# BienLuky/Rectified-SpaAttn

Measured on AMD Instinct MI355X. Metric: attention-layer TFLOPs/sec (rectified block-sparse attention, HunyuanVideo seq~120k d=128 bf16), higher is better.
Workload: dtype bf16; 1 GPU; hunyuan_720p_128f: B=1 H=24 S=115456 (115200 visual + 256 text, 200 valid) D=128, top_k=90, regime=r2 (p_remain=0.0, neighbors=none); heads_per_gpu=24, parallelism=head-shard x1, world_size=1

## Files before the change

### rectified_spaattn_amd/csrc/rsa_attn.h

```cpp
#pragma once
#include <string.h>

#include <type_traits>

#include "rsa_common.h"

typedef short s16x4 __attribute__((ext_vector_type(4)));
typedef short s16x8 __attribute__((ext_vector_type(8)));
typedef __bf16 bf16x8 __attribute__((ext_vector_type(8)));
typedef _Float16 f16x8 __attribute__((ext_vector_type(8)));
typedef float f32x16 __attribute__((ext_vector_type(16)));
typedef float f32x4 __attribute__((ext_vector_type(4)));

template <typename Tag>
struct Elem;
template <>
struct Elem<bf16_tag> {
    static __device__ __forceinline__ f32x16 mfma(s16x8 a, s16x8 b, f32x16 c) {
        return __builtin_amdgcn_mfma_f32_32x32x16_bf16(__builtin_bit_cast(bf16x8, a), __builtin_bit_cast(bf16x8, b),
                                                       c, 0, 0, 0);
    }
    static __device__ __forceinline__ unsigned short from_f32(float f) {
        return __builtin_bit_cast(unsigned short, (__bf16)f);
    }
    static __device__ __forceinline__ s16x8 cvt8(const float* f) {
        bf16x8 r;
#pragma unroll
        for (int i = 0; i < 8; ++i) r[i] = (__bf16)f[i];
        return __builtin_bit_cast(s16x8, r);
    }
};
template <>
struct Elem<fp16_tag> {
    static __device__ __forceinline__ f32x16 mfma(s16x8 a, s16x8 b, f32x16 c) {
        return __builtin_amdgcn_mfma_f32_32x32x16_f16(__builtin_bit_cast(f16x8, a), __builtin_bit_cast(f16x8, b), c,
                                                      0, 0, 0);
    }
    static __device__ __forceinline__ unsigned short from_f32(float f) {
        return __builtin_bit_cast(unsigned short, (_Float16)f);
    }
    static __device__ __forceinline__ s16x8 cvt8(const float* f) {
        f16x8 r;
#pragma unroll
        for (int i = 0; i < 8; ++i) r[i] = (_Float16)f[i];
        return __builtin_bit_cast(s16x8, r);
    }
};

enum { MODE_SPARSE = 0, MODE_DENSE = 1 };

struct WalkArgs {
    unsigned short* out;
    long osb, osh, oss;
    const int32_t* cols;
    const int32_t* counts;
    const float* R;
    const float* comp;
    float* tpart;
    float* tail_part;
    unsigned* gsync;
    int mode, H, Sq, Sk;
    int NBv, NQB, NB_total;
    int kv_valid, kv_text_valid, q_text_end;
    int q_split, kv_split;
    int causal;
    int n_heavy_pad, NBp, BH;
    int tsplit, tper;
    int heavy_last;
    int tail_first, tail_n, tail_p;
    int gsync_gen;
    int gsync_ratio;
    int k5_static;
};

struct AttnArgs : WalkArgs {
    const unsigned short *q, *k, *v;
    long qsb, qsh, qss, ksb, ksh, kss, vsb, vsh, vss;
    float qk_scale;
    int rows256;
    int blk;
    int txt0;
    const int32_t* row_lo;
    const int32_t* row_hi;
    long range_sb;
    int kv_group, list_group, gqa;
};
enum { RSA_GQA_NONE = 0, RSA_GQA_HEAD = 1, RSA_GQA_PAIR = 2 };

template <typename A>
__device__ __forceinline__ const A& rsa_kernargs() {
    return *static_cast<const A*>((const void*)__builtin_amdgcn_kernarg_segment_ptr());
}

__host__ __device__ __forceinline__ int rsa_walk_unit(int j, int NBp) { return (j & 7) * (NBp >> 3) + (j >> 3); }
enum { WALK_NONE = 0, WALK_SPARSE = 1, WALK_TEXT = 2 };
__device__ __forceinline__ int rsa_walk_map(const WalkArgs& a, int work, int n_units, int& bh, int& unit, int& tsp, int& tail) {
    tsp = 0;
    tail = -1;
    const int n_sparse = a.BH * a.NBp;
    const bool heavy_last = a.heavy_last != 0;
    int wh = heavy_last ? work - n_sparse : work;
    int v = heavy_last ? work : work - a.n_heavy_pad;
    bool text = heavy_last ? work >= n_sparse : work < a.n_heavy_pad;
    if (a.tail_n > 0) {
        const int tail_end = a.tail_first + a.tail_n * a.tail_p;
        text = work >= tail_end;
        wh = work - tail_end;
        if (work >= a.tail_first && !text) {
            tail = work - a.tail_first;
            v = a.tail_first + tail / a.tail_p;
            tsp = tail % a.tail_p;
        }
    }
    if (text) {
        const int ntq = a.NQB - a.NBv;
        const int per_bh = ntq * a.tsplit;
        if (ntq <= 0 || wh >= a.BH * per_bh) return WALK_NONE;
        bh = wh / per_bh;
        const int rem = wh % per_bh;
        unit = a.NBv + rem / a.tsplit;
        tsp = rem % a.tsplit;
    } else {
        bh = v / a.NBp;
        unit = rsa_walk_unit(v % a.NBp, a.NBp);
        if (unit >= n_units) return WALK_NONE;
    }
    return text ? WALK_TEXT : WALK_SPARSE;
}

__device__ __forceinline__ void rsa_walk_list(const WalkArgs& a, long rowi, int tail, int tsp, const int32_t*& list, int& n_items) {
    list = a.cols + rowi * a.NB_total;
    n_items = a.counts[rowi];
    if (tail >= 0) {
        const int per = (n_items + a.tail_p - 1) / a.tail_p, first = tsp * per;
        const int left = n_items - first;
        list += first;
        n_items = left < 0 ? 0 : (left < per ? left : per);
    }
}
__device__ __forceinline__ void rsa_walk_text(const WalkArgs& a, int blk, int tsp, int& first_blk, int& n_items) {
    n_items = (a.kv_text_valid + blk - 1) / blk;
    if (a.tsplit > 1) {
        first_blk = tsp * a.tper;
        n_items = n_items - first_blk < a.tper ? n_items - first_blk : a.tper;
        if (n_items < 0) n_items = 0;
    }
}

__device__ __forceinline__ int rsa_seg_hi(const WalkArgs& a, int row) {
    const bool s1 = row >= a.q_split;
    const int lo = s1 ? a.kv_split : 0, hi = s1 ? a.Sk : a.kv_split;
    if (!a.causal) return hi;
    const int rows = s1 ? a.Sq - a.q_split : a.q_split, rin = row - (s1 ? a.q_split : 0);
    const int lim = lo + rin + 1 + ((hi - lo) - rows);
    return lim < lo ? lo : (lim < hi ? lim : hi);
}
__device__ __forceinline__ void rsa_dense_row(const WalkArgs& a, int grow, int& lo, int& hi) {
    lo = grow < a.q_split ? 0 : a.kv_split;
    hi = rsa_seg_hi(a, grow < a.Sq ? grow : a.Sq - 1);
}
__device__ __forceinline__ void rsa_dense_tile(const WalkArgs& a, int row0, int rows, int& lo_max, int& hi_min, int& hi_max,
                                               int& first_blk, int& n_items) {
    const int row1 = row0 + rows;
    int lo_min;
    const int rlast = (row1 <= a.Sq ? row1 : a.Sq) - 1;
    if (row1 <= a.q_split) { lo_min = 0; lo_max = 0; }
    else if (row0 >= a.q_split) { lo_min = lo_max = a.kv_split; }
    else { lo_min = 0; lo_max = a.kv_split; }
    hi_min = rsa_seg_hi(a, row0);
    hi_max = rsa_seg_hi(a, rlast);
    if (row0 < a.q_split && rlast >= a.q_split) {
        const int h0 = rsa_seg_hi(a, a.q_split - 1), h1 = rsa_seg_hi(a, a.q_split);
        hi_min = hi_min < h1 ? hi_min : h1;
        hi_max = hi_max > h0 ? hi_max : h0;
    }
    first_blk = lo_min / RSA_BLOCK;
    n_items = (hi_max + RSA_BLOCK - 1) / RSA_BLOCK - first_blk;
    if (hi_max <= lo_min) n_items = 0;
}

// ... 79 lines not shown
```

### rectified_spaattn_amd/csrc/rsa_attn.hip

```cpp
#include <stdlib.h>

#include <atomic>
#include <mutex>
#include "rsa_attn.h"

static int g_k5_tsplit = 1;
extern int g_rsa_k3_prefix;
extern int g_rsa_k3_long;
extern int g_rsa_k4_split;
extern int g_rsa_k2_dma;
static int g_k5_tail_split = 1;
static int g_k5_text_last = 1;
static int g_shard_invariant = 0;
static int g_k5_gsync_ratio = 2;
int rsa_gsync_ratio() { return g_k5_gsync_ratio; }
static int g_k5_rows256 = 1;
static int g_k5_static = 1;
int rsa_k5_static() { return g_k5_static; }
static int g_k5_gqa_pair = 0;
static int g_k5_gsync = 1;

extern "C" int rsa_set_tuning(const char* key, int value) {
    static const bool enabled = [] { const char* e = getenv("RSA_TUNING"); return e && e[0] == '1'; }();
    if (!key) return RSA_ERR_BAD_ARG;
    if (!enabled) return RSA_ERR_UNSUPPORTED;
    if (strcmp(key, "k3_prefix") == 0) { g_rsa_k3_prefix = value; return RSA_OK; }
    if (strcmp(key, "k3_long") == 0) { g_rsa_k3_long = value; return RSA_OK; }
    if (strcmp(key, "k4_split") == 0) { g_rsa_k4_split = value; return RSA_OK; }
    if (strcmp(key, "k2_dma") == 0) { g_rsa_k2_dma = value; return RSA_OK; }
    if (strcmp(key, "k5_static") == 0) { g_k5_static = value; return RSA_OK; }
    if (strcmp(key, "k5_rows256") == 0) { g_k5_rows256 = value; return RSA_OK; }
    if (strcmp(key, "k5_tsplit") == 0) { g_k5_tsplit = value; return RSA_OK; }
    if (strcmp(key, "k5_gsync") == 0) { g_k5_gsync = value; return RSA_OK; }
    if (strcmp(key, "k5_gsync_ratio") == 0) { g_k5_gsync_ratio = value; return RSA_OK; }
    if (strcmp(key, "k5_text_last") == 0) { g_k5_text_last = value; return RSA_OK; }
    if (strcmp(key, "k5_tail_split") == 0) { g_k5_tail_split = value; return RSA_OK; }
    if (strcmp(key, "k5_gqa_pair") == 0) { g_k5_gqa_pair = value; return RSA_OK; }
    if (strcmp(key, "fp8_variant") == 0) { rsa_set_fp8_variant(value); return RSA_OK; }
    if (strcmp(key, "fp8_smooth_k") == 0) { rsa_set_fp8_smooth_k(value); return RSA_OK; }
    return RSA_ERR_BAD_ARG;
}

template <typename Tag>
__global__ __launch_bounds__(256) void text_combine_kernel(const float* __restrict__ tpart, unsigned short* out,
                                                           long osb, long osh, long oss, int D, int H, int txt0, int ntq,
                                                           int tsplit, int q_text_end, int Sq, long rows_total) {
    const int lane = threadIdx.x & 63;
    const long row = (long)blockIdx.x * 4 + (threadIdx.x >> 6);
    if (row >= rows_total) return;
    const long bhq = row / RSA_BLOCK;
    const int r = (int)(row % RSA_BLOCK);
    const long bh = bhq / ntq;
    const int tq = (int)(bhq % ntq);
    const int grow = txt0 + tq * RSA_BLOCK + r;
    if (grow >= Sq) return;
    const float* base = tpart + rsa_part_row(bhq * tsplit, r, D);
    const long pstride = rsa_part_row(1, 0, D);
    constexpr int MAXP = RSA_TEXT_SPLIT;
    float mv[MAXP], lv[MAXP];
#pragma unroll
    for (int s = 0; s < MAXP; ++s) {
        const int sc = s < tsplit ? s : 0;
        const float2 ml = *reinterpret_cast<const float2*>(base + sc * pstride + D);
        mv[s] = s < tsplit ? ml.x : -INFINITY;
        lv[s] = ml.y;
    }
    float M = -INFINITY;
#pragma unroll
    for (int s = 0; s < MAXP; ++s) M = fmaxf(M, mv[s]);
    float L = 0.0f;
    float acc[2] = {0.0f, 0.0f};
#pragma unroll
    for (int s0 = 0; s0 < MAXP; s0 += 8) {
        if (s0 >= tsplit) break;
        float x[8][2];
#pragma unroll
        for (int u = 0; u < 8; ++u) {
            const int sc = s0 + u < tsplit ? s0 + u : 0;
#pragma unroll
            for (int e = 0; e < 2; ++e) {
                const int d = lane + 64 * e;
                x[u][e] = d < D ? base[sc * pstride + d] : 0.0f;
            }
        }
#pragma unroll
        for (int u = 0; u < 8; ++u) {
            if (s0 + u < tsplit) {
                const float wgt = (mv[s0 + u] == -INFINITY) ? 0.0f : __builtin_amdgcn_exp2f(mv[s0 + u] - M);
                L += lv[s0 + u] * wgt;
// ... 77 lines not shown
        text_combine_kernel<fp16_tag><<<grid, 256, 0, s>>>(a.tpart, a.out, a.osb, a.osh, a.oss, D, a.H, a.NBv * blk, ntq, a.tsplit,
                                                         a.q_text_end, a.Sq, rows);
    return rsa_launch_status();
}

__device__ unsigned g_rsa_gsync[RSA_GSYNC_RING][RSA_GSYNC_SLOT_WORDS];
unsigned* rsa_gsync_slot(int which, unsigned grid, int wg_per_cu, hipStream_t s, int* gen) {
    static std::atomic<unsigned*> base[64];
    static std::atomic<unsigned> ticket{0};
    *gen = 32 * (wg_per_cu > 0 ? wg_per_cu : 2);
    if (!(g_k5_gsync & which) || wg_per_cu <= 0 || grid <= 16u * (unsigned)*gen) return nullptr;
    const unsigned gens = ((grid + 7) / 8 + *gen - 1) / *gen;
    int dev = -1;
    if (gens > RSA_GSYNC_MAXG || hipGetDevice(&dev) != hipSuccess || dev < 0 || dev >= 64) return nullptr;
    unsigned* b = base[dev].load();
    if (!b) {
        int cus = 0;
        if (hipDeviceGetAttribute(&cus, hipDeviceAttributeMultiprocessorCount, dev) != hipSuccess || cus != 256) {
            base[dev].store(reinterpret_cast<unsigned*>(1));
            return nullptr;
        }
        if (hipGetSymbolAddress(reinterpret_cast<void**>(&b), HIP_SYMBOL(g_rsa_gsync)) != hipSuccess) return nullptr;
        base[dev].store(b);
    }
    if (b == reinterpret_cast<unsigned*>(1)) return nullptr;
    unsigned* slot = b + (size_t)(ticket.fetch_add(1) % RSA_GSYNC_RING) * RSA_GSYNC_SLOT_WORDS;
    return hipMemsetAsync(slot, 0, (8 + 8 * (size_t)gens) * sizeof(unsigned), s) == hipSuccess ? slot : nullptr;
}
int rsa_wg_per_cu(const void* kernel, int block, size_t lds_bytes) {
    struct Entry { const void* k; size_t lds; int dev, n; };
    static Entry cache[64];
    static std::atomic<int> used{0};
    static std::mutex mu;
    int dev = -1;
    if (hipGetDevice(&dev) != hipSuccess) return 0;
    const int nu = used.load(std::memory_order_acquire);
    for (int i = 0; i < nu; ++i)
        if (cache[i].k == kernel && cache[i].lds == lds_bytes && cache[i].dev == dev) return cache[i].n;
    int n = 0;
    if (hipOccupancyMaxActiveBlocksPerMultiprocessor(&n, kernel, block, lds_bytes) != hipSuccess) n = 0;
    std::lock_guard<std::mutex> lk(mu);
    const int at = used.load();
    if (at < 64) { cache[at] = Entry{kernel, lds_bytes, dev, n}; used.store(at + 1, std::memory_order_release); }
    return n;
}

int rsa_plan_walk(WalkArgs& a, int BH, int D, const WalkPolicy& pol, size_t tpart_bytes, long* nblocks) {
    *nblocks = 0;
    const int blk = pol.blk;
    const int ntq = a.NQB - a.NBv;
    if (a.tpart && tpart_bytes == 0) return RSA_ERR_WORKSPACE;
    const size_t piece_bytes = (size_t)rsa_part_row(1, 0, D) * sizeof(float);
    a.BH = BH;
    a.NBp = ((blk == 64 ? (a.NBv + 1) >> 1 : a.NBv) + 7) & ~7;
    const int n_txt_items = (a.kv_text_valid + blk - 1) / blk;
    a.tsplit = 1; a.tper = n_txt_items;
    if (a.mode == MODE_SPARSE && ntq > 0 && a.tpart && g_k5_tsplit && n_txt_items >= 32) {
        const int sp = n_txt_items / 16;
        int cap = ((long)BH * a.NBp < 8 * 512 && !g_shard_invariant) ? pol.short_grid_text_cap : 16;
        const size_t room = tpart_bytes / ((size_t)BH * (size_t)ntq * piece_bytes);
        if ((size_t)cap > room) cap = (int)room;
        a.tsplit = sp > cap ? cap : sp;
        if (a.tsplit < 2) a.tsplit = 1;
        a.tper = (n_txt_items + a.tsplit - 1) / a.tsplit;
    }
    const int n_heavy = ntq > 0 ? BH * ntq * a.tsplit : 0;
    a.heavy_last = a.tsplit > 1 && g_k5_text_last;
    a.n_heavy_pad = (n_heavy + 7) & ~7;
    const long n_sparse = (long)BH * a.NBp;
    *nblocks = (long)a.n_heavy_pad + n_sparse;
    a.tail_first = a.tail_n = a.tail_p = 0; a.tail_part = nullptr;
    if (pol.tail_split && a.mode == MODE_SPARSE && a.tpart && (n_heavy == 0 || (pol.tail_beside_text && a.heavy_last)) && g_k5_tail_split &&
        !g_shard_invariant) {
        const long full = n_sparse / 512, T = n_sparse % 512;
        const long room = 512 - a.n_heavy_pad;
        const long P = T > 0 ? (room / T < 4 ? room / T : 4) : 0;
        const size_t text_pieces = (size_t)BH * (size_t)ntq * RSA_TEXT_SPLIT;
        if (full >= 1 && T > 0 && P >= 2 && (text_pieces + (size_t)(T * P)) * piece_bytes <= tpart_bytes) {
            a.tail_first = (int)(full * 512); a.tail_n = (int)T; a.tail_p = (int)P;
            a.tail_part = a.tpart + rsa_part_row((long)text_pieces, 0, D);
            *nblocks = (long)a.tail_first + (long)a.tail_n * a.tail_p + a.n_heavy_pad;
        }
    }
    if (*nblocks <= 0) { *nblocks = 0; return RSA_OK; }
    if (*nblocks > 0x7FFFFFFF) return RSA_ERR_UNSUPPORTED;
    if (a.NB_total > 8192) return RSA_ERR_UNSUPPORTED;
    return RSA_OK;
}

static int launch_attn(AttnArgs& a, int BH, int D, int dtype, size_t tpart_bytes, hipStream_t s) {
    const bool w64 = a.blk == RSA_BLOCK;
    long nblocks;
    WalkPolicy pol;
    pol.blk = a.blk;
    pol.short_grid_text_cap = RSA_TEXT_SPLIT;
    pol.tail_split = w64 && D == 128 && a.gqa != RSA_GQA_PAIR;
    pol.tail_beside_text = true;
    int st = rsa_plan_walk(a, BH, D, pol, tpart_bytes, &nblocks);
    if (st != RSA_OK || nblocks == 0) return st;
    const size_t lds_bytes = (size_t)4 * 64 * D * 2 + (((size_t)a.NB_total * 2 + 15) & ~(size_t)15);
    st = w64 ? rsa_launch_bsfwd64(a, dim3((unsigned)nblocks), lds_bytes, D, dtype, s)
             : rsa_launch_bsfwd(a, dim3((unsigned)nblocks), lds_bytes, D, dtype, s);
    return st != RSA_OK ? st : rsa_combine_walk(a, D, a.blk, dtype, s);
}

static void fill_qkv(AttnArgs& a, const rsa_tensor4& q, const rsa_tensor4& k, const rsa_tensor4& v,
                     const rsa_out4& out) {
    a.q = static_cast<const unsigned short*>(q.ptr); a.qsb = q.stride_b; a.qsh = q.stride_h; a.qss = q.stride_s;
    a.k = static_cast<const unsigned short*>(k.ptr); a.ksb = k.stride_b; a.ksh = k.stride_h; a.kss = k.stride_s;
    a.v = static_cast<const unsigned short*>(v.ptr); a.vsb = v.stride_b; a.vsh = v.stride_h; a.vss = v.stride_s;
    a.out = static_cast<unsigned short*>(out.ptr); a.osb = out.stride_b; a.osh = out.stride_h; a.oss = out.stride_s;
    a.row_lo = nullptr; a.row_hi = nullptr; a.range_sb = 0;
    a.kv_group = 1; a.list_group = 1; a.gqa = RSA_GQA_NONE;
}

int rsa_check_out(const rsa_out4& o) {
    if (!o.ptr || (reinterpret_cast<uintptr_t>(o.ptr) & 7)) return RSA_ERR_BAD_ARG;
    if ((o.stride_b % 4) || (o.stride_h % 4) || (o.stride_s % 4)) return RSA_ERR_BAD_ARG;
    return RSA_OK;
}

static int block_sparse_fwd_b(const rsa_layout* l, int blk, rsa_tensor4 q, rsa_tensor4 k, rsa_tensor4 v,
                              const rsa_buffers* buf, rsa_out4 out, void* stream) {
    int st = rsa_check_layout_b(l, blk);
    if (st != RSA_OK) return st;
    if ((st = rsa_check_tensor(q)) || (st = rsa_check_tensor(k)) || (st = rsa_check_tensor(v)) ||
        (st = rsa_check_out(out)))
        return st;
    if (!buf || (l->NBv > 0 && (!buf->cols || !buf->counts))) return RSA_ERR_BAD_ARG;
    if ((buf->R == nullptr) != (buf->comp == nullptr)) return RSA_ERR_BAD_ARG;
    AttnArgs a;
    fill_qkv(a, q, k, v, out);
    a.cols = buf->cols; a.counts = buf->counts; a.R = buf->R; a.comp = buf->comp;
    a.tpart = buf->tpart;
    a.mode = MODE_SPARSE; a.H = l->H; a.Sq = l->S; a.Sk = l->S;
    a.NBv = l->NBv; a.NQB = l->NB_total; a.NB_total = l->NB_total;
    a.blk = blk; a.txt0 = l->NBv * blk;
    if (blk == 64) a.NQB = l->NBv + (l->NB_total - l->NBv + 1) / 2;
    a.kv_valid = l->kv_valid; a.kv_text_valid = l->kv_text_valid;
    a.q_text_end = l->NBv * blk + l->q_text_valid;
    a.q_split = 0; a.kv_split = 0; a.causal = 0; a.rows256 = 0;
    a.qk_scale = (float)((1.0 / sqrt((double)l->D)) * 1.44269504);
    return launch_attn(a, l->B * l->H, l->D, l->dtype, buf->tpart_bytes, static_cast<hipStream_t>(stream));
}
extern "C" int rsa_block_sparse_fwd(const rsa_layout* l, rsa_tensor4 q, rsa_tensor4 k, rsa_tensor4 v,
                                    const rsa_buffers* buf, rsa_out4 out, void* stream) {
    return block_sparse_fwd_b(l, RSA_BLOCK, q, k, v, buf, out, stream);
}
extern "C" int rsa_block_sparse_fwd_ex(const rsa_layout_ex* lx, rsa_tensor4 q, rsa_tensor4 k, rsa_tensor4 v,
                                       const rsa_buffers* buf, rsa_out4 out, void* stream) {
    return rsa_layout_ex_ok(lx) ? block_sparse_fwd_b(&lx->base, lx->block, q, k, v, buf, out, stream) : RSA_ERR_BAD_ARG;
}
// ... 139 lines not shown
```

### rectified_spaattn_amd/csrc/rsa_attn_kernel64.hip

```cpp
#include "rsa_attn.h"
#include <atomic>
#include "rsa_attn_block64.h"

#define RSA_K5W_CL_TO RSA_K5W_CLOBBER_TMP, RSA_K5W_CLOBBER_O
#define RSA_K5V_CL_TO RSA_K5V_CLOBBER_TMP, RSA_K5V_CLOBBER_O
#define RSA_K5W_CL_LOOP RSA_K5W_CLOBBER_TMP, RSA_K5W_CLOBBER_O, RSA_K5W_CLOBBER_LOOP
#define RSA_K5V_CL_LOOP RSA_K5V_CLOBBER_TMP, RSA_K5V_CLOBBER_O, RSA_K5V_CLOBBER_LOOP
#define RSA_K5_ASM(D_, BODY, OPS, CL, ...) \
    do { \
        if constexpr ((D_) == 128) asm volatile(RSA_K5W_##BODY RSA_K5W_##OPS : RSA_K5W_##CL __VA_ARGS__); \
        else asm volatile(RSA_K5V_##BODY RSA_K5V_##OPS : RSA_K5V_##CL __VA_ARGS__); \
    } while (0)

typedef int i32x8 __attribute__((ext_vector_type(8)));
typedef unsigned u32x4 __attribute__((ext_vector_type(4)));

__device__ __forceinline__ int k5w_max(int x, int y) { return x > y ? x : y; }
__device__ __forceinline__ int k5w_wave_max(int v) {
#pragma unroll
    for (int m = 32; m >= 1; m >>= 1) v = k5w_max(v, __shfl_xor(v, m, 64));
    return v;
}

template <typename Tag, int U, int D>
__device__ __forceinline__ void k5w_block(f32x16 (&SA)[2], f32x16 (&SB)[2], const f32x16 (&nm)[2], float (&l)[2], float (&mx)[2],
                                          const i32x8& ka, const i32x8& va) {
    if constexpr (std::is_same<Tag, bf16_tag>::value) {
        if constexpr (U == 0) RSA_K5_ASM(D, BLOCK_BF16_U0, OPS, CL_TO, , "memory");
        else if constexpr (U == 1) RSA_K5_ASM(D, BLOCK_BF16_U1, OPS, CL_TO, , "memory");
        else if constexpr (U == 2) RSA_K5_ASM(D, BLOCK_BF16_U2, OPS, CL_TO, , "memory");
        else RSA_K5_ASM(D, BLOCK_BF16_U3, OPS, CL_TO, , "memory");
    } else {
        if constexpr (U == 0) RSA_K5_ASM(D, BLOCK_F16_U0, OPS, CL_TO, , "memory");
        else if constexpr (U == 1) RSA_K5_ASM(D, BLOCK_F16_U1, OPS, CL_TO, , "memory");
        else if constexpr (U == 2) RSA_K5_ASM(D, BLOCK_F16_U2, OPS, CL_TO, , "memory");
        else RSA_K5_ASM(D, BLOCK_F16_U3, OPS, CL_TO, , "memory");
    }
}

template <int Hh, int KSI, int D>
__device__ __forceinline__ void k5w_qwrite(const s16x8& f) {
#define RSA_QW(HH, KK) do { if constexpr (D == 128) asm volatile(RSA_K5W_QWRITE_H##HH##_K##KK :: "{v[96:99]}"(f) : RSA_K5W_CLOBBER_Q); \
                            else asm volatile(RSA_K5V_QWRITE_H##HH##_K##KK :: "{v[96:99]}"(f) : RSA_K5V_CLOBBER_Q); } while (0)
    if constexpr (Hh == 0) {
        if constexpr (KSI == 0) RSA_QW(0, 0); else if constexpr (KSI == 1) RSA_QW(0, 1); else if constexpr (KSI == 2) RSA_QW(0, 2);
        else if constexpr (KSI == 3) RSA_QW(0, 3); else if constexpr (KSI == 4) RSA_QW(0, 4); else if constexpr (KSI == 5) RSA_QW(0, 5);
        else if constexpr (KSI == 6) RSA_QW(0, 6); else RSA_QW(0, 7);
    } else {
        if constexpr (KSI == 0) RSA_QW(1, 0); else if constexpr (KSI == 1) RSA_QW(1, 1); else if constexpr (KSI == 2) RSA_QW(1, 2);
        else if constexpr (KSI == 3) RSA_QW(1, 3); else if constexpr (KSI == 4) RSA_QW(1, 4); else if constexpr (KSI == 5) RSA_QW(1, 5);
        else if constexpr (KSI == 6) RSA_QW(1, 6); else RSA_QW(1, 7);
    }
#undef RSA_QW
}
template <int Hh, int DTI, int D>
__device__ __forceinline__ f32x16 k5w_oread() {
    f32x16 t;
#define RSA_OR(HH, DD) do { if constexpr (D == 128) asm volatile(RSA_K5W_OREAD_H##HH##_D##DD : "={v[96:111]}"(t)); \
                            else asm volatile(RSA_K5V_OREAD_H##HH##_D##DD : "={v[96:111]}"(t)); } while (0)
    if constexpr (Hh == 0) {
        if constexpr (DTI == 0) RSA_OR(0, 0); else if constexpr (DTI == 1) RSA_OR(0, 1); else if constexpr (DTI == 2) RSA_OR(0, 2); else RSA_OR(0, 3);
    } else {
        if constexpr (DTI == 0) RSA_OR(1, 0); else if constexpr (DTI == 1) RSA_OR(1, 1); else if constexpr (DTI == 2) RSA_OR(1, 2); else RSA_OR(1, 3);
    }
#undef RSA_OR
    return t;
}

template <typename Tag, bool WIDE, int NW = 2, int D = 128, bool RANGED = false, int GQA = RSA_GQA_NONE>
__global__ __launch_bounds__(64 * NW) __attribute__((amdgpu_waves_per_eu(1, 1))) void bsfwd64_kernel(AttnArgs) {
    constexpr bool PAIR = GQA == RSA_GQA_PAIR;
    static_assert(!RANGED || NW == 2 || PAIR, "per-row ranges: sparse calls only (128-row query blocks)");
    static_assert(PAIR ? NW == 4 : (GQA == RSA_GQA_NONE || NW == 2), "a head pair is four waves, a head of its own two");
    const AttnArgs& a = rsa_kernargs<AttnArgs>();
    constexpr int RW = PAIR ? 128 : 64 * NW;
    constexpr int NPIECE = 32 * D * 2 / 1024;
    constexpr int NPW = NPIECE / NW;
    constexpr int RPP = 32 / NPIECE;
    constexpr int LPR = 64 / RPP;
    static_assert(NW == 2 || NW == 4, "two or four waves");
    constexpr int KS = D / 16;
    constexpr int DT = D / 32;
    constexpr int HALF = 32 * D * 2;
    constexpr int VRING = 4 * HALF;
    using E = Elem<Tag>;
    extern __shared__ __attribute__((aligned(16))) unsigned char lds[];
    unsigned short* lds_list = reinterpret_cast<unsigned short*>(lds + 8 * HALF);
    __shared__ int redo_flag;

    const GsyncTicket gs_tk = rsa_gsync_announce(a.gsync, a.gsync_gen);

    int bh, qblk, tsp, tail;
    if (rsa_walk_map(a, blockIdx.x, a.NBv, bh, qblk, tsp, tail) == WALK_NONE) return;
    int b = bh / a.H, h = bh % a.H;
    const int t = threadIdx.x, lane = t & 63;
    const int wv = __builtin_amdgcn_readfirstlane(t >> 6);
    int wq = wv;
    if constexpr (PAIR) {
        const int hp = a.H >> 1;
        b = bh / hp; h = 2 * (bh % hp) + (wv >> 1); wq = wv & 1;
    }
    const int r = lane & 31, hh = lane >> 5;
    int grow[2];
    grow[0] = qblk * RW + 64 * wq + r;
    grow[1] = grow[0] + 32;

    int lo_r[2] = {0, 0}, hi_r[2] = {0, 0};
    int n_items, first_blk = 0, lo_max, hi_min, hi_max;
    const int32_t* list = nullptr;
    if (a.mode == MODE_SPARSE) {
        if (qblk < a.NBv) {
            long lrow = bh;
            if constexpr (GQA != RSA_GQA_NONE) lrow = (long)b * (a.H / a.list_group) + h / a.list_group;
            rsa_walk_list(a, lrow * a.NBv + qblk, tail, tsp, list, n_items);
            if constexpr (RANGED) {
                const int32_t* lo_p = a.row_lo ? a.row_lo + (long)b * a.range_sb : nullptr;
                const int32_t* hi_p = a.row_hi + (long)b * a.range_sb;
                const int kvv = a.kv_valid;
                int red4[4] = {-kvv, 0, -kvv, 0};
#pragma unroll
                for (int x = 0; x < 2; ++x) {
                    const int row = grow[x] < a.Sq ? grow[x] : a.Sq - 1;
                    int lo = lo_p ? lo_p[row] : 0, hi = hi_p[row];
                    lo = lo < 0 ? 0 : (lo < kvv ? lo : kvv);
                    hi = hi < 0 ? 0 : (hi < kvv ? hi : kvv);
                    const bool none = hi <= lo;
                    lo_r[x] = none ? 0 : lo;
                    hi_r[x] = none ? 0 : hi;
                    red4[0] = k5w_max(red4[0], none ? -kvv : -lo);
                    red4[1] = k5w_max(red4[1], lo_r[x]);
                    red4[2] = k5w_max(red4[2], -hi_r[x]);
                    red4[3] = k5w_max(red4[3], hi_r[x]);
                }
                int* red = reinterpret_cast<int*>(lds);
#pragma unroll
                for (int i = 0; i < 4; ++i) {
                    const int m = k5w_wave_max(red4[i]);
                    if (lane == 0) red[4 * wv + i] = m;
                }
                __syncthreads();
                int lo_min;
                if constexpr (NW == 2) {
                    lo_min = -__builtin_amdgcn_readfirstlane(k5w_max(red[0], red[4]));
                    lo_max = __builtin_amdgcn_readfirstlane(k5w_max(red[1], red[5]));
                    hi_min = -__builtin_amdgcn_readfirstlane(k5w_max(red[2], red[6]));
                    hi_max = __builtin_amdgcn_readfirstlane(k5w_max(red[3], red[7]));
// ... 218 lines not shown
        rescale_check(I0{}, mxA, SA, SB, nm);
        const unsigned cnt = (unsigned)(i1 - i0);
        const unsigned blk0 = cnt ? (unsigned)blk_of(i0) : 0u, blk1 = cnt ? (unsigned)blk_of(i0 + 1) : 0u;
        unsigned la = lds_base + 8 * HALF + 2 * (i0 + 2), lv;
        const unsigned long kb = (unsigned long)(uintptr_t)kbase, vb = (unsigned long)(uintptr_t)vbase;
        const unsigned ldsk = lds_base + wv * 1024, ldsv = lds_base + VRING + wv * 1024;
        float (&l)[2] = l_run;
        float (&mx)[2] = mxA;
        unsigned stat = 0;
        if (may_static && pass == 0 && cnt != 0 &&
            __builtin_amdgcn_ballot_w64(thr[0] == -INFINITY || thr[1] == -INFINITY) == 0ull) stat = 1;
        stat = __builtin_amdgcn_readfirstlane(stat);
        used_static = stat != 0;
        if constexpr (NW == 4 && std::is_same<Tag, bf16_tag>::value) RSA_K5_ASM(D, LOOP_BF16_R256, OPS_LOOP, CL_LOOP, , "memory");
        else if constexpr (NW == 4) RSA_K5_ASM(D, LOOP_F16_R256, OPS_LOOP, CL_LOOP, , "memory");
        else if constexpr (std::is_same<Tag, bf16_tag>::value) RSA_K5_ASM(D, LOOP_BF16, OPS_LOOP, CL_LOOP, , "memory");
        else RSA_K5_ASM(D, LOOP_F16, OPS_LOOP, CL_LOOP, , "memory");
        (void)lv;
    }
    run_items(i1, n_items);
    if (!may_static) break;
    {
        asm volatile("s_nop 11" ::: "memory");
        unsigned emax = 0;
        auto track = [&](const f32x16& o) {
#pragma unroll
            for (int i = 0; i < 16; ++i) {
                const unsigned bits = __float_as_uint(o[i]) & 0x7FFFFFFFu;
                emax = emax > bits ? emax : bits;
            }
        };
        if (used_static) {
            track(k5w_oread<0, 0, D>()); track(k5w_oread<0, 1, D>()); track(k5w_oread<1, 0, D>()); track(k5w_oread<1, 1, D>());
            if constexpr (DT == 4) {
                track(k5w_oread<0, 2, D>()); track(k5w_oread<0, 3, D>()); track(k5w_oread<1, 2, D>()); track(k5w_oread<1, 3, D>());
            }
        }
        const bool lbad = (__float_as_uint(l_run[0]) & 0x7FFFFFFFu) >= 0x71800000u || (__float_as_uint(l_run[1]) & 0x7FFFFFFFu) >= 0x71800000u;
        const bool bad = used_static && (emax >= 0x7F800000u || lbad);
        if (__builtin_amdgcn_ballot_w64(bad) != 0ull && lane == 0) redo_flag = 1;
        __syncthreads();
        if (redo_flag == 0) break;
    }
    }

    asm volatile("s_nop 11" ::: "memory");
    const AttnArgs* ep = &rsa_kernargs<AttnArgs>();
    asm volatile("" : "+s"(ep));
    const AttnArgs& e = *ep;
    int bh2, qblk2, tsp2, tail2;
    {
        int work2 = blockIdx.x;
        asm volatile("" : "+s"(work2));
        rsa_walk_map(e, work2, e.NBv, bh2, qblk2, tsp2, tail2);
    }
    int b2, h2;
    if constexpr (PAIR) {
        const int hp2 = e.H >> 1;
        b2 = bh2 / hp2; h2 = 2 * (bh2 % hp2) + (wv >> 1);
    } else {
        b2 = bh2 / e.H; h2 = bh2 % e.H;
    }
    const bool partial = (e.mode == MODE_SPARSE && e.tsplit > 1 && qblk2 >= e.NBv) || tail2 >= 0;
    const bool rectify = e.mode == MODE_SPARSE && qblk2 < e.NBv && e.R != nullptr && tail2 < 0;
    float4 cv[DT][4];
    float Rv = 1.0f;
#pragma unroll
    for (int dt = 0; dt < DT; ++dt)
#pragma unroll
        for (int g = 0; g < 4; ++g) cv[dt][g] = make_float4(0, 0, 0, 0);
    if (rectify) {
        const long rowi = (long)bh2 * e.NBv + qblk2;
        const float* cp = e.comp + rowi * D;
#pragma unroll
        for (int dt = 0; dt < DT; ++dt)
#pragma unroll
            for (int g = 0; g < 4; ++g) cv[dt][g] = *reinterpret_cast<const float4*>(cp + 32 * dt + 8 * g + 4 * hh);
        Rv = e.R[rowi];
    }
    auto finish_half = [&](auto HX) {
        constexpr int x = decltype(HX)::value;
        const int grow2 = qblk2 * RW + 64 * wq + 32 * x + r;
        const float mrun = thr[x] == -INFINITY ? -INFINITY : m_ref[x];
        const auto swl = __builtin_amdgcn_permlane32_swap(__float_as_uint(l_run[x]), __float_as_uint(l_run[x]), false, false);
        const float l_tot = __uint_as_float(swl[0]) + __uint_as_float(swl[1]);
        if (partial) {
            float* pp = rsa_part_of(e, bh2, qblk2, tsp2, tail2, 64 * wq + 32 * x + r, D);
            auto put = [&](int dt, const f32x16& o) {
#pragma unroll
                for (int g = 0; g < 4; ++g) {
                    const int d0 = 32 * dt + 8 * g + 4 * hh;
                    *reinterpret_cast<float2*>(pp + d0) = make_float2(o[4 * g + 0], o[4 * g + 1]);
                    *reinterpret_cast<float2*>(pp + d0 + 2) = make_float2(o[4 * g + 2], o[4 * g + 3]);
                }
            };
            put(0, k5w_oread<x, 0, D>()); put(1, k5w_oread<x, 1, D>());
            if constexpr (DT == 4) { put(2, k5w_oread<x, 2, D>()); put(3, k5w_oread<x, 3, D>()); }
            if (hh == 0) *reinterpret_cast<float2*>(pp + D) = make_float2(mrun, l_tot);
            return;
        }
        const bool text_blk = e.mode == MODE_SPARSE && qblk2 >= e.NBv;
        const bool st_r = grow2 < (text_blk ? e.q_text_end : e.Sq);
        const bool zr = text_blk && !st_r && grow2 < e.Sq;
        if (!(st_r || zr)) return;
        float inv = l_tot > 0.0f ? 1.0f / l_tot : 0.0f;
        if (zr) inv = 0.0f;
        const float sc = inv * Rv;
// ... 16 lines not shown
                        const float v0 = fin(o[4 * g + 0], c4.x);
                        const float v1 = fin(o[4 * g + 1], c4.y);
                        const float v2 = fin(o[4 * g + 2], c4.z);
                        const float v3 = fin(o[4 * g + 3], c4.w);
                        pk[gi].x = (unsigned)E::from_f32(v0) | ((unsigned)E::from_f32(v1) << 16);
                        pk[gi].y = (unsigned)E::from_f32(v2) | ((unsigned)E::from_f32(v3) << 16);
                    }
                    const auto sx = __builtin_amdgcn_permlane32_swap(pk[0].x, pk[1].x, false, false);
                    const auto sy = __builtin_amdgcn_permlane32_swap(pk[0].y, pk[1].y, false, false);
                    uint4 w4;
                    w4.x = sx[0]; w4.y = sy[0]; w4.z = sx[1]; w4.w = sy[1];
                    *reinterpret_cast<uint4*>(op + 32 * dt + 8 * (2 * gp + hh)) = w4;
                }
            } else {
#pragma unroll
                for (int g = 0; g < 4; ++g) {
                    const int d0 = 32 * dt + 8 * g + 4 * hh;
                    float4 c4 = cv[dt][g];
                    if (zr) c4 = make_float4(0, 0, 0, 0);
                    const float v0 = fin(o[4 * g + 0], c4.x);
                    const float v1 = fin(o[4 * g + 1], c4.y);
                    const float v2 = fin(o[4 * g + 2], c4.z);
                    const float v3 = fin(o[4 * g + 3], c4.w);
                    uint2 pk;
                    pk.x = (unsigned)E::from_f32(v0) | ((unsigned)E::from_f32(v1) << 16);
                    pk.y = (unsigned)E::from_f32(v2) | ((unsigned)E::from_f32(v3) << 16);
                    *reinterpret_cast<uint2*>(op + d0) = pk;
                }
            }
        };
        put(0, k5w_oread<x, 0, D>()); put(1, k5w_oread<x, 1, D>());
        if constexpr (DT == 4) { put(2, k5w_oread<x, 2, D>()); put(3, k5w_oread<x, 3, D>()); }
    };
    finish_half(std::integral_constant<int, 0>{});
    finish_half(std::integral_constant<int, 1>{});
}

template <int NW, int D, bool RANGED = false, int GQA = RSA_GQA_NONE>
static int launch_bsfwd64(const AttnArgs& a, bool wide, int dtype, dim3 grid, size_t lds_bytes, hipStream_t s) {
    const bool sparse = a.mode == MODE_SPARSE;
    if (dtype == RSA_BF16) {
        if (wide) RSA_LAUNCH_GSYNC(1, (bsfwd64_kernel<bf16_tag, true, NW, D, RANGED, GQA>), a, sparse, grid, 64 * NW, lds_bytes, s);
        else RSA_LAUNCH_GSYNC(1, (bsfwd64_kernel<bf16_tag, false, NW, D, RANGED, GQA>), a, sparse, grid, 64 * NW, lds_bytes, s);
    } else {
        if (wide) RSA_LAUNCH_GSYNC(1, (bsfwd64_kernel<fp16_tag, true, NW, D, RANGED, GQA>), a, sparse, grid, 64 * NW, lds_bytes, s);
        else RSA_LAUNCH_GSYNC(1, (bsfwd64_kernel<fp16_tag, false, NW, D, RANGED, GQA>), a, sparse, grid, 64 * NW, lds_bytes, s);
    }
    return rsa_launch_status();
}

#ifndef RSA_K64_GQA_UNIT
int rsa_launch_bsfwd64(const AttnArgs& a, dim3 grid, size_t lds_bytes, int D, int dtype, hipStream_t s) {
    if (D != 128 && D != 64) return RSA_ERR_UNSUPPORTED;
    const bool wide = !(((uintptr_t)a.out & 15) || ((a.osb | a.osh | a.oss) & 7));
    lds_bytes += 16;
    if (a.gqa != RSA_GQA_NONE) return rsa_launch_bsfwd64_gqa(a, wide, grid, lds_bytes, D, dtype, s);
    if (a.rows256) {
        if (a.mode != MODE_DENSE) return RSA_ERR_BAD_ARG;
        return D == 128 ? launch_bsfwd64<4, 128>(a, wide, dtype, grid, lds_bytes, s) : launch_bsfwd64<4, 64>(a, wide, dtype, grid, lds_bytes, s);
    }
    if (a.row_hi) {
        if (a.mode != MODE_SPARSE) return RSA_ERR_BAD_ARG;
        return D == 128 ? launch_bsfwd64<2, 128, true>(a, wide, dtype, grid, lds_bytes, s)
                        : launch_bsfwd64<2, 64, true>(a, wide, dtype, grid, lds_bytes, s);
    }
    return D == 128 ? launch_bsfwd64<2, 128>(a, wide, dtype, grid, lds_bytes, s) : launch_bsfwd64<2, 64>(a, wide, dtype, grid, lds_bytes, s);
}
#else
template <int NW, int GQA>
static int launch_gqa(const AttnArgs& a, bool wide, dim3 grid, size_t lds_bytes, int D, int dtype, hipStream_t s) {
    if (a.row_hi)
        return D == 128 ? launch_bsfwd64<NW, 128, true, GQA>(a, wide, dtype, grid, lds_bytes, s)
                        : launch_bsfwd64<NW, 64, true, GQA>(a, wide, dtype, grid, lds_bytes, s);
    return D == 128 ? launch_bsfwd64<NW, 128, false, GQA>(a, wide, dtype, grid, lds_bytes, s)
                    : launch_bsfwd64<NW, 64, false, GQA>(a, wide, dtype, grid, lds_bytes, s);
}
#if RSA_K64_GQA_UNIT == 1
static_assert(RSA_GQA_HEAD == 1, "RSA_K64_GQA_UNIT names the form");
int rsa_launch_bsfwd64_gqa(const AttnArgs& a, bool wide, dim3 grid, size_t lds_bytes, int D, int dtype, hipStream_t s) {
    if (a.mode != MODE_SPARSE || a.rows256 || a.kv_group <= 0 || a.list_group <= 0) return RSA_ERR_BAD_ARG;
    if (a.gqa == RSA_GQA_PAIR) return rsa_launch_bsfwd64_gqa_pair(a, wide, grid, lds_bytes, D, dtype, s);
    return launch_gqa<2, RSA_GQA_HEAD>(a, wide, grid, lds_bytes, D, dtype, s);
}
#else
static_assert(RSA_K64_GQA_UNIT == RSA_GQA_PAIR, "RSA_K64_GQA_UNIT names the form");
int rsa_launch_bsfwd64_gqa_pair(const AttnArgs& a, bool wide, dim3 grid, size_t lds_bytes, int D, int dtype, hipStream_t s) {
    if ((a.kv_group | a.list_group | a.H) & 1) return RSA_ERR_BAD_ARG;
    return launch_gqa<4, RSA_GQA_PAIR>(a, wide, grid, lds_bytes, D, dtype, s);
}
#endif
#endif
```

Measured before the change: 1185 TFLOP/s.

## Reorder sparse query-block walk by mean KV-column key for L2 locality

Adds two pre-pass kernels. The first computes a mean-column sort key for each query block, along with its list overlap with the next block. The second bitonic-sorts the blocks per head into a walk order stored in the tpart workspace. The attention kernel then maps work items through this order, grouped per XCD and gsync generation, so that blocks with similar KV lists run close in time and share L2. If average neighbour overlap already exceeds a threshold, identity order is kept. The cost is two extra launches and an indirection on every sparse work item.

```diff
diff --git a/rectified_spaattn_amd/csrc/rsa_attn.h b/rectified_spaattn_amd/csrc/rsa_attn.h
--- a/rectified_spaattn_amd/csrc/rsa_attn.h
+++ b/rectified_spaattn_amd/csrc/rsa_attn.h
@@ -4,6 +4,7 @@
 #include <type_traits>
 
 #include "rsa_common.h"
+#include "rsa_walk_order.h"
 
 typedef short s16x4 __attribute__((ext_vector_type(4)));
 typedef short s16x8 __attribute__((ext_vector_type(8)));
@@ -71,6 +72,7 @@
     int gsync_gen;
     int gsync_ratio;
     int k5_static;
+    const unsigned short* order;
 };
 
 struct AttnArgs : WalkArgs {
@@ -92,40 +94,9 @@
     return *static_cast<const A*>((const void*)__builtin_amdgcn_kernarg_segment_ptr());
 }
 
-__host__ __device__ __forceinline__ int rsa_walk_unit(int j, int NBp) { return (j & 7) * (NBp >> 3) + (j >> 3); }
-enum { WALK_NONE = 0, WALK_SPARSE = 1, WALK_TEXT = 2 };
+template <bool ORDERED = false>
 __device__ __forceinline__ int rsa_walk_map(const WalkArgs& a, int work, int n_units, int& bh, int& unit, int& tsp, int& tail) {
-    tsp = 0;
-    tail = -1;
-    const int n_sparse = a.BH * a.NBp;
-    const bool heavy_last = a.heavy_last != 0;
-    int wh = heavy_last ? work - n_sparse : work;
-    int v = heavy_last ? work : work - a.n_heavy_pad;
-    bool text = heavy_last ? work >= n_sparse : work < a.n_heavy_pad;
-    if (a.tail_n > 0) {
-        const int tail_end = a.tail_first + a.tail_n * a.tail_p;
-        text = work >= tail_end;
-        wh = work - tail_end;
-        if (work >= a.tail_first && !text) {
-            tail = work - a.tail_first;
-            v = a.tail_first + tail / a.tail_p;
-            tsp = tail % a.tail_p;
-        }
-    }
-    if (text) {
-        const int ntq = a.NQB - a.NBv;
-        const int per_bh = ntq * a.tsplit;
-        if (ntq <= 0 || wh >= a.BH * per_bh) return WALK_NONE;
-        bh = wh / per_bh;
-        const int rem = wh % per_bh;
-        unit = a.NBv + rem / a.tsplit;
-        tsp = rem % a.tsplit;
-    } else {
-        bh = v / a.NBp;
-        unit = rsa_walk_unit(v % a.NBp, a.NBp);
-        if (unit >= n_units) return WALK_NONE;
-    }
-    return text ? WALK_TEXT : WALK_SPARSE;
+    return rsa_walk_map_t<ORDERED>(a, work, n_units, bh, unit, tsp, tail);
 }
 
 __device__ __forceinline__ void rsa_walk_list(const WalkArgs& a, long rowi, int tail, int tsp, const int32_t*& list, int& n_items) {
diff --git a/rectified_spaattn_amd/csrc/rsa_attn.hip b/rectified_spaattn_amd/csrc/rsa_attn.hip
--- a/rectified_spaattn_amd/csrc/rsa_attn.hip
+++ b/rectified_spaattn_amd/csrc/rsa_attn.hip
@@ -18,6 +18,8 @@
 static int g_k5_static = 1;
 int rsa_k5_static() { return g_k5_static; }
 static int g_k5_gqa_pair = 0;
+static int g_k5_walk_order = 1;
+static int g_k5_order_overlap = 50;
 static int g_k5_gsync = 1;
 
 extern "C" int rsa_set_tuning(const char* key, int value) {
@@ -35,6 +37,8 @@
     if (strcmp(key, "k5_gsync_ratio") == 0) { g_k5_gsync_ratio = value; return RSA_OK; }
     if (strcmp(key, "k5_text_last") == 0) { g_k5_text_last = value; return RSA_OK; }
     if (strcmp(key, "k5_tail_split") == 0) { g_k5_tail_split = value; return RSA_OK; }
+    if (strcmp(key, "k5_walk_order") == 0) { g_k5_walk_order = value; return RSA_OK; }
+    if (strcmp(key, "k5_order_overlap") == 0) { g_k5_order_overlap = value; return RSA_OK; }
     if (strcmp(key, "k5_gqa_pair") == 0) { g_k5_gqa_pair = value; return RSA_OK; }
     if (strcmp(key, "fp8_variant") == 0) { rsa_set_fp8_variant(value); return RSA_OK; }
     if (strcmp(key, "fp8_smooth_k") == 0) { rsa_set_fp8_smooth_k(value); return RSA_OK; }
@@ -218,6 +222,7 @@
     if (a.tpart && tpart_bytes == 0) return RSA_ERR_WORKSPACE;
     const size_t piece_bytes = (size_t)rsa_part_row(1, 0, D) * sizeof(float);
     a.BH = BH;
+    a.order = nullptr;
     a.NBp = ((blk == 64 ? (a.NBv + 1) >> 1 : a.NBv) + 7) & ~7;
     const int n_txt_items = (a.kv_text_valid + blk - 1) / blk;
     a.tsplit = 1; a.tper = n_txt_items;
@@ -254,6 +259,129 @@
     return RSA_OK;
 }
 
+
+constexpr int ORD_NT = 1024, ORD_BM_WORDS = 8192 / 32, ORD_UNIT_NT = 256;
+constexpr unsigned ORD_KEY_EMPTY = 0x7FFFEu;
+__device__ __forceinline__ int ord_wave_sum(int x) {
+    x += __builtin_amdgcn_update_dpp(0, x, 0xB1, 0xF, 0xF, false);
+    x += __builtin_amdgcn_update_dpp(0, x, 0x4E, 0xF, 0xF, false);
+    x += __builtin_amdgcn_update_dpp(0, x, 0x124, 0xF, 0xF, false);
+    x += __builtin_amdgcn_update_dpp(0, x, 0x128, 0xF, 0xF, false);
+    return __builtin_amdgcn_readlane(x, 0) + __builtin_amdgcn_readlane(x, 16) + __builtin_amdgcn_readlane(x, 32) +
+           __builtin_amdgcn_readlane(x, 48);
+}
+__device__ __forceinline__ void ord_wave_sync() {
+    __builtin_amdgcn_fence(__ATOMIC_SEQ_CST, "wavefront");
+    __builtin_amdgcn_wave_barrier();
+}
+__global__ __launch_bounds__(ORD_UNIT_NT) void walk_order_unit_kernel(const int32_t* __restrict__ cols, const int32_t* __restrict__ counts,
+                                                                      unsigned* __restrict__ ukey, float* __restrict__ uovl, int BH,
+                                                                      int NBv, int NBp, int NB_total) {
+    __shared__ unsigned ord_bm[ORD_UNIT_NT / 64][ORD_BM_WORDS];
+    const int lane = threadIdx.x & 63, wv = threadIdx.x >> 6;
+    const long w = (long)blockIdx.x * (ORD_UNIT_NT / 64) + wv;
+    if (w >= (long)BH * NBv) return;
+    const int bh = (int)(w / NBv), i = (int)(w % NBv);
+    unsigned* bm = ord_bm[wv];
+    const long row = (long)bh * NBv + i;
+    const bool has_next = i + 1 < NBv;
+    const int32_t* la = cols + row * NB_total;
+    const int32_t* lb = la + (has_next ? NB_total : 0);
+    const int a0 = lane < NB_total ? la[lane] : -1, a1 = lane + 64 < NB_total ? la[lane + 64] : -1;
+    const int b0 = lane < NB_total ? lb[lane] : -1, b1 = lane + 64 < NB_total ? lb[lane + 64] : -1;
+    int na = counts[row], nb = has_next ? counts[row + 1] : 0;
+    na = na < 0 ? 0 : (na < NB_total ? na : NB_total);
+    nb = nb < 0 ? 0 : (nb < NB_total ? nb : NB_total);
+    for (int x = lane; x < ORD_BM_WORDS; x += 64) bm[x] = 0u;
+    ord_wave_sync();
+    for (int x = lane; x < nb; x += 64) {
+        const int e = x < 64 ? b0 : (x < 128 ? b1 : lb[x]);
+        if ((unsigned)e < (unsigned)NB_total) atomicOr(&bm[e >> 5], 1u << (e & 31));
+    }
+    ord_wave_sync();
+    int sum = 0, hit = 0;
+    for (int x = lane; x < na; x += 64) {
+        const int e = x < 64 ? a0 : (x < 128 ? a1 : la[x]);
+        if ((unsigned)e < (unsigned)NB_total) {
+            sum += e;
+            hit += (int)((bm[e >> 5] >> (e & 31)) & 1u);
+        }
+    }
+    sum = ord_wave_sum(sum);
+    hit = ord_wave_sum(hit);
+    if (lane == 0) {
+        const unsigned key = na > 0 ? ((unsigned)sum << 6) / (unsigned)na : ORD_KEY_EMPTY;
+        ukey[(long)bh * NBp + i] = (key << 13) | (unsigned)i;
+        uovl[(long)bh * NBp + i] = (has_next && na > 0) ? (float)hit / (float)na : -1.0f;
+    }
+}
+__global__ __launch_bounds__(ORD_NT) void walk_order_sort_kernel(const unsigned* __restrict__ ukey, const float* __restrict__ uovl,
+                                                                 unsigned short* __restrict__ order, int NBv, int NBp, int P2,
+                                                                 int n_whole, int thr_pct) {
+    extern __shared__ unsigned ord_keys[];
+    __shared__ float ord_ov[ORD_NT / 64];
+    __shared__ int ord_np[ORD_NT / 64];
+    __shared__ int ord_identity;
+    const int bh = blockIdx.x, t = threadIdx.x, lane = t & 63, wv = t >> 6;
+    const long left = (long)n_whole - (long)bh * NBp;
+    const int r0 = left < 0 ? 0 : (left < NBp ? (int)left : NBp);
+    const unsigned key_t = t < NBv ? ukey[(long)bh * NBp + t] : 0u;
+    float ov = 0.0f;
+    int np = 0;
+    for (int i = t; i < NBv; i += ORD_NT) {
+        const float o = uovl[(long)bh * NBp + i];
+        if (o >= 0.0f) { ov += o; ++np; }
+    }
+    for (int m = 1; m < 64; m <<= 1) { ov += __shfl_xor(ov, m, 64); np += __shfl_xor(np, m, 64); }
+    if (lane == 0) { ord_ov[wv] = ov; ord_np[wv] = np; }
+    __syncthreads();
+    if (t == 0) {
+        float so = 0.0f;
+        int sp = 0;
+        for (int w = 0; w < ORD_NT / 64; ++w) { so += ord_ov[w]; sp += ord_np[w]; }
+        ord_identity = so * 100.0f >= (float)thr_pct * (float)sp;
+    }
+    __syncthreads();
+    const bool identity = ord_identity != 0;
+    for (int i = t; i < P2; i += ORD_NT) {
+        unsigned key = 0xFFFFFFFFu;
+        if (i < NBv && rsa_walk_unit_inv(i, NBp) < r0) key = identity ? (unsigned)i : (i == t ? key_t : ukey[(long)bh * NBp + i]);
+        ord_keys[i] = key;
+    }
+    __syncthreads();
+    for (int k = 2; k <= P2; k <<= 1) {
+        for (int j = k >> 1; j >= 64; j >>= 1) {
+            for (int i = t; i < P2; i += ORD_NT) {
+                const int x = i ^ j;
+                if (x > i) {
+                    const unsigned ka = ord_keys[i], kb = ord_keys[x];
+                    if ((ka > kb) == ((i & k) == 0)) { ord_keys[i] = kb; ord_keys[x] = ka; }
+                }
+            }
+            __syncthreads();
+        }
+        for (int i0 = 0; i0 < P2; i0 += ORD_NT) {
+            const int i = i0 + t;
+            unsigned key = i < P2 ? ord_keys[i] : 0xFFFFFFFFu;
+            for (int j = k >> 1 < 32 ? k >> 1 : 32; j > 0; j >>= 1) {
+                const unsigned other = (unsigned)__shfl_xor((int)key, j, 64);
+                const bool low = (i & j) == 0, up = (i & k) == 0;
+                const unsigned mn = key < other ? key : other, mx = key < other ? other : key;
+                key = (low == up) ? mn : mx;
+            }
+            if (i < P2) ord_keys[i] = key;
+        }
+        __syncthreads();
+    }
+    unsigned short* o = order + (long)bh * NBp;
+    for (int r = t; r < NBp; r += ORD_NT) {
+        int u;
+        if (r < r0) u = (r < P2 && ord_keys[r] != 0xFFFFFFFFu) ? (int)(ord_keys[r] & 0x1FFFu) : RSA_ORDER_PAD;
+        else u = rsa_walk_unit(r, NBp);
+        o[r] = (unsigned short)(u < NBv ? u : RSA_ORDER_PAD);
+    }
+}
+
 static int launch_attn(AttnArgs& a, int BH, int D, int dtype, size_t tpart_bytes, hipStream_t s) {
     const bool w64 = a.blk == RSA_BLOCK;
     long nblocks;
@@ -264,6 +392,29 @@
     pol.tail_beside_text = true;
     int st = rsa_plan_walk(a, BH, D, pol, tpart_bytes, &nblocks);
     if (st != RSA_OK || nblocks == 0) return st;
+    if (g_k5_walk_order && w64 && a.mode == MODE_SPARSE && a.gqa == RSA_GQA_NONE && !a.row_hi && a.tpart && a.NBv > 0 &&
+        a.NBv <= 8192 && (a.heavy_last || a.n_heavy_pad == 0)) {
+        const int ntq = a.NQB - a.NBv;
+        const size_t piece_bytes = (size_t)rsa_part_row(1, 0, D) * sizeof(float);
+        const size_t used = ((size_t)BH * (size_t)(ntq > 0 ? ntq : 0) * RSA_TEXT_SPLIT + (size_t)a.tail_n * (size_t)a.tail_p) * piece_bytes;
+        const size_t n_ent = (size_t)BH * (size_t)a.NBp;
+        const size_t need = n_ent * (sizeof(unsigned short) + sizeof(unsigned) + sizeof(float));
+        if (used <= tpart_bytes && need <= tpart_bytes - used) {
+            char* base = reinterpret_cast<char*>(a.tpart) + used;
+            unsigned short* order = reinterpret_cast<unsigned short*>(base);
+            unsigned* ukey = reinterpret_cast<unsigned*>(base + n_ent * sizeof(unsigned short));
+            float* uovl = reinterpret_cast<float*>(ukey + n_ent);
+            int P2 = 1;
+            while (P2 < a.NBv) P2 <<= 1;
+            const long waves = (long)BH * a.NBv, per_wg = ORD_UNIT_NT / 64;
+            walk_order_unit_kernel<<<dim3((unsigned)((waves + per_wg - 1) / per_wg)), ORD_UNIT_NT, 0, s>>>(a.cols, a.counts, ukey, uovl, BH, a.NBv,
+                                                                                                        a.NBp, a.NB_total);
+            walk_order_sort_kernel<<<dim3((unsigned)BH), ORD_NT, (size_t)P2 * sizeof(unsigned), s>>>(
+                ukey, uovl, order, a.NBv, a.NBp, P2, a.tail_n > 0 ? a.tail_first : (int)n_ent, g_k5_order_overlap);
+            if ((st = rsa_launch_status()) != RSA_OK) return st;
+            a.order = order;
+        }
+    }
     const size_t lds_bytes = (size_t)4 * 64 * D * 2 + (((size_t)a.NB_total * 2 + 15) & ~(size_t)15);
     st = w64 ? rsa_launch_bsfwd64(a, dim3((unsigned)nblocks), lds_bytes, D, dtype, s)
              : rsa_launch_bsfwd(a, dim3((unsigned)nblocks), lds_bytes, D, dtype, s);
diff --git a/rectified_spaattn_amd/csrc/rsa_attn_kernel64.hip b/rectified_spaattn_amd/csrc/rsa_attn_kernel64.hip
--- a/rectified_spaattn_amd/csrc/rsa_attn_kernel64.hip
+++ b/rectified_spaattn_amd/csrc/rsa_attn_kernel64.hip
@@ -70,6 +70,7 @@
 template <typename Tag, bool WIDE, int NW = 2, int D = 128, bool RANGED = false, int GQA = RSA_GQA_NONE>
 __global__ __launch_bounds__(64 * NW) __attribute__((amdgpu_waves_per_eu(1, 1))) void bsfwd64_kernel(AttnArgs) {
     constexpr bool PAIR = GQA == RSA_GQA_PAIR;
+    constexpr bool ORDERED = NW == 2 && !RANGED && GQA == RSA_GQA_NONE;
     static_assert(!RANGED || NW == 2 || PAIR, "per-row ranges: sparse calls only (128-row query blocks)");
     static_assert(PAIR ? NW == 4 : (GQA == RSA_GQA_NONE || NW == 2), "a head pair is four waves, a head of its own two");
     const AttnArgs& a = rsa_kernargs<AttnArgs>();
@@ -91,7 +92,7 @@
     const GsyncTicket gs_tk = rsa_gsync_announce(a.gsync, a.gsync_gen);
 
     int bh, qblk, tsp, tail;
-    if (rsa_walk_map(a, blockIdx.x, a.NBv, bh, qblk, tsp, tail) == WALK_NONE) return;
+    if (rsa_walk_map<ORDERED>(a, blockIdx.x, a.NBv, bh, qblk, tsp, tail) == WALK_NONE) return;
     int b = bh / a.H, h = bh % a.H;
     const int t = threadIdx.x, lane = t & 63;
     const int wv = __builtin_amdgcn_readfirstlane(t >> 6);
@@ -416,7 +417,7 @@
     {
         int work2 = blockIdx.x;
         asm volatile("" : "+s"(work2));
-        rsa_walk_map(e, work2, e.NBv, bh2, qblk2, tsp2, tail2);
+        rsa_walk_map<ORDERED>(e, work2, e.NBv, bh2, qblk2, tsp2, tail2);
     }
     int b2, h2;
     if constexpr (PAIR) {
@@ -539,6 +540,7 @@
 #ifndef RSA_K64_GQA_UNIT
 int rsa_launch_bsfwd64(const AttnArgs& a, dim3 grid, size_t lds_bytes, int D, int dtype, hipStream_t s) {
     if (D != 128 && D != 64) return RSA_ERR_UNSUPPORTED;
+    if (a.order && (a.gqa != RSA_GQA_NONE || a.rows256 || a.row_hi)) return RSA_ERR_BAD_ARG;
     const bool wide = !(((uintptr_t)a.out & 15) || ((a.osb | a.osh | a.oss) & 7));
     lds_bytes += 16;
     if (a.gqa != RSA_GQA_NONE) return rsa_launch_bsfwd64_gqa(a, wide, grid, lds_bytes, D, dtype, s);
diff --git a/rectified_spaattn_amd/csrc/rsa_walk_order.h b/rectified_spaattn_amd/csrc/rsa_walk_order.h
--- /dev/null
+++ b/rectified_spaattn_amd/csrc/rsa_walk_order.h
@@ -0,0 +1,64 @@
+#pragma once
+
+#if defined(__HIPCC__)
+#define RSA_WALK_FN __host__ __device__ __forceinline__
+#else
+#define RSA_WALK_FN static inline
+#endif
+
+enum { WALK_NONE = 0, WALK_SPARSE = 1, WALK_TEXT = 2 };
+enum { RSA_ORDER_PAD = 0xFFFF };
+
+RSA_WALK_FN int rsa_walk_unit(int j, int NBp) { return (j & 7) * (NBp >> 3) + (j >> 3); }
+RSA_WALK_FN int rsa_walk_unit_inv(int unit, int NBp) { return (unit % (NBp >> 3)) * 8 + unit / (NBp >> 3); }
+
+RSA_WALK_FN int rsa_walk_pos(int v, int n_whole, int gen) {
+    const int per = 8 * gen;
+    if (v >= n_whole / per * per) return v;
+    const int xcd = v & 7, n = v >> 3, g = n / gen, i = n % gen;
+    return (g * 8 + xcd) * gen + i;
+}
+
+RSA_WALK_FN int rsa_walk_sparse(const unsigned short* order, int v, int n_whole, int NBp, int gen, int& bh) {
+    if (!order || v >= n_whole) {
+        bh = v / NBp;
+        return rsa_walk_unit(v % NBp, NBp);
+    }
+    const int p = rsa_walk_pos(v, n_whole, gen);
+    bh = p / NBp;
+    return order[p];
+}
+
+template <bool ORDERED, typename A>
+RSA_WALK_FN int rsa_walk_map_t(const A& a, int work, int n_units, int& bh, int& unit, int& tsp, int& tail) {
+    tsp = 0;
+    tail = -1;
+    const int n_sparse = a.BH * a.NBp;
+    const bool heavy_last = a.heavy_last != 0;
+    int wh = heavy_last ? work - n_sparse : work;
+    int v = heavy_last ? work : work - a.n_heavy_pad;
+    bool text = heavy_last ? work >= n_sparse : work < a.n_heavy_pad;
+    if (a.tail_n > 0) {
+        const int tail_end = a.tail_first + a.tail_n * a.tail_p;
+        text = work >= tail_end;
+        wh = work - tail_end;
+        if (work >= a.tail_first && !text) {
+            tail = work - a.tail_first;
+            v = a.tail_first + tail / a.tail_p;
+            tsp = tail % a.tail_p;
+        }
+    }
+    if (text) {
+        const int ntq = a.NQB - a.NBv;
+        const int per_bh = ntq * a.tsplit;
+        if (ntq <= 0 || wh >= a.BH * per_bh) return WALK_NONE;
+        bh = wh / per_bh;
+        const int rem = wh % per_bh;
+        unit = a.NBv + rem / a.tsplit;
+        tsp = rem % a.tsplit;
+    } else {
+        unit = rsa_walk_sparse(ORDERED ? a.order : nullptr, v, a.tail_n > 0 ? a.tail_first : n_sparse, a.NBp, a.gsync_gen, bh);
+        if (unit >= n_units) return WALK_NONE;
+    }
+    return text ? WALK_TEXT : WALK_SPARSE;
+}
```

Result: faster. 1223 TFLOP/s, median of 6 (+3.2%).
